# Drexubery/ViewCrafter

Measured on NVIDIA H100. Metric: DDIM denoise-steps/sec @ 576x1024x25f, higher is better.
Workload: dtype f16 (fp32 accumulate; fp32 norms/softmax/update)

## Files before the change

viewcrafter_b200/csrc/common.cuh:

```cuda
#pragma once
#include <cuda.h>
#include <cuda_fp16.h>
#include <cuda_runtime.h>
#include <stdint.h>

#define VC_OK 0
#define VC_ERR_ARG 1
#define VC_ERR_CUDA 2
#define VC_ERR_UNSUPPORTED 3

namespace vc {

void set_error(const char* fmt, ...);
const char* last_error();

#define VC_CHECK_CUDA(expr)                                                                      \
  do {                                                                                           \
    cudaError_t _e = (expr);                                                                     \
    if (_e != cudaSuccess) {                                                                     \
      vc::set_error("%s failed: %s (%s:%d)", #expr, cudaGetErrorString(_e), __FILE__, __LINE__); \
      return VC_ERR_CUDA;                                                                        \
    }                                                                                            \
  } while (0)

#define VC_REQUIRE(cond, ...)       \
  do {                              \
    if (!(cond)) {                  \
      vc::set_error(__VA_ARGS__);   \
      return VC_ERR_ARG;            \
    }                               \
  } while (0)

int encode_tmap_f16(CUtensorMap* out, const void* base, int rank, const uint64_t* dims,
                    const uint64_t* strides_bytes, const uint32_t* box, int swizzle_bytes = 128);

int sm_count();

struct DeviceOnce {
  unsigned long long done[4] = {0, 0, 0, 0};
};
bool device_once_needed(DeviceOnce& o);
void device_once_mark(DeviceOnce& o);

#ifdef __CUDACC__

__device__ __forceinline__ uint32_t smem_u32(const void* p) { return (uint32_t)__cvta_generic_to_shared(p); }

__device__ __forceinline__ bool elect_one() {
  uint32_t pred = 0;
  asm volatile(
      "{\n\t.reg .pred P1;\n\t.reg .b32 R1;\n\t"
      "elect.sync R1|P1, 0xffffffff;\n\t"
      "selp.b32 %0, 1, 0, P1;\n\t}\n"
      : "=r"(pred));
  return pred != 0;
}

__device__ __forceinline__ void mbar_init(uint64_t* bar, uint32_t count) {
  asm volatile("mbarrier.init.shared::cta.b64 [%0], %1;" ::"r"(smem_u32(bar)), "r"(count) : "memory");
}
__device__ __forceinline__ void fence_barrier_init() {
  asm volatile("fence.mbarrier_init.release.cluster;" ::: "memory");
}
__device__ __forceinline__ void fence_proxy_async() {
  asm volatile("fence.proxy.async.shared::cta;" ::: "memory");
}
__device__ __forceinline__ void mbar_expect_tx(uint64_t* bar, uint32_t bytes) {
  asm volatile("mbarrier.arrive.expect_tx.shared::cta.b64 _, [%0], %1;" ::"r"(smem_u32(bar)), "r"(bytes) : "memory");
}
__device__ __forceinline__ void mbar_arrive(uint64_t* bar) {
  asm volatile("mbarrier.arrive.shared::cta.b64 _, [%0];" ::"r"(smem_u32(bar)) : "memory");
}
__device__ __forceinline__ bool mbar_try_wait(uint64_t* bar, uint32_t parity) {
  uint32_t ok;
  asm volatile(
      "{\n\t.reg .pred P1;\n\t"
      "mbarrier.try_wait.parity.shared::cta.b64 P1, [%1], %2;\n\t"
      "selp.b32 %0, 1, 0, P1;\n\t}\n"
      : "=r"(ok)
      : "r"(smem_u32(bar)), "r"(parity)
      : "memory");
  return ok != 0;
}
__device__ __forceinline__ void mbar_wait(uint64_t* bar, uint32_t parity) {
  while (!mbar_try_wait(bar, parity)) {
  }
}
__device__ __forceinline__ void tma_prefetch_desc(const CUtensorMap* m) {
  asm volatile("prefetch.tensormap [%0];" ::"l"(reinterpret_cast<uint64_t>(m)) : "memory");
}
__device__ __forceinline__ void tma_load_2d(void* dst, const CUtensorMap* m, uint64_t* bar, int c0, int c1) {
  asm volatile(
      "cp.async.bulk.tensor.2d.shared::cta.global.mbarrier::complete_tx::bytes [%0], [%1, {%3, %4}], [%2];" ::"r"(smem_u32(dst)),
      "l"(reinterpret_cast<uint64_t>(m)), "r"(smem_u32(bar)), "r"(c0), "r"(c1)
      : "memory");
}
__device__ __forceinline__ void tma_load_4d(void* dst, const CUtensorMap* m, uint64_t* bar, int c0, int c1, int c2, int c3) {
  asm volatile(
      "cp.async.bulk.tensor.4d.shared::cta.global.mbarrier::complete_tx::bytes [%0], [%1, {%3, %4, %5, %6}], [%2];" ::"r"(smem_u32(dst)),
      "l"(reinterpret_cast<uint64_t>(m)), "r"(smem_u32(bar)), "r"(c0), "r"(c1), "r"(c2), "r"(c3)
      : "memory");
}
__device__ __forceinline__ void tma_store_4d(const CUtensorMap* m, const void* src, int c0, int c1, int c2, int c3) {
  asm volatile("cp.async.bulk.tensor.4d.global.shared::cta.bulk_group [%0, {%2, %3, %4, %5}], [%1];" ::"l"(reinterpret_cast<uint64_t>(m)),
               "r"(smem_u32(src)), "r"(c0), "r"(c1), "r"(c2), "r"(c3)
               : "memory");
}
__device__ __forceinline__ void tma_store_3d(const CUtensorMap* m, const void* src, int c0, int c1, int c2) {
  asm volatile("cp.async.bulk.tensor.3d.global.shared::cta.bulk_group [%0, {%2, %3, %4}], [%1];" ::"l"(reinterpret_cast<uint64_t>(m)),
               "r"(smem_u32(src)), "r"(c0), "r"(c1), "r"(c2)
               : "memory");
}
__device__ __forceinline__ void tma_store_commit() { asm volatile("cp.async.bulk.commit_group;" ::: "memory"); }
__device__ __forceinline__ void tma_store_wait_read() { asm volatile("cp.async.bulk.wait_group.read 0;" ::: "memory"); }
__device__ __forceinline__ void tma_store_wait_all() { asm volatile("cp.async.bulk.wait_group 0;" ::: "memory"); }
__device__ __forceinline__ void fence_proxy_async_smem() { asm volatile("fence.proxy.async.shared::cta;" ::: "memory"); }

__device__ __forceinline__ void wgmma_fence() { asm volatile("wgmma.fence.sync.aligned;" ::: "memory"); }
__device__ __forceinline__ void wgmma_commit() { asm volatile("wgmma.commit_group.sync.aligned;" ::: "memory"); }
template <int N>
__device__ __forceinline__ void wgmma_wait() { asm volatile("wgmma.wait_group.sync.aligned %0;" ::"n"(N) : "memory"); }
template <int R>
__device__ __forceinline__ void wgmma_fence_regs(float (&d)[R]) {
#pragma unroll
  for (int i = 0; i < R; ++i) asm volatile("" : "+f"(d[i])::"memory");
}
__device__ __forceinline__ void named_bar_sync(int id, int count) { asm volatile("bar.sync %0, %1;" ::"r"(id), "r"(count) : "memory"); }

__device__ __forceinline__ uint64_t wgmma_desc_sw128(uint32_t smem_addr, uint32_t lbo_bytes = 16, uint32_t sbo_bytes = 1024) {
  uint64_t d = 0;
  d |= (uint64_t)((smem_addr & 0x3FFFF) >> 4);
  d |= (uint64_t)((lbo_bytes >> 4) & 0x3FFF) << 16;
  d |= (uint64_t)((sbo_bytes >> 4) & 0x3FFF) << 32;
  d |= (uint64_t)1 << 62;
  return d;
}

__device__ __forceinline__ uint32_t pack_half2(float a, float b) {
  __half2 h = __floats2half2_rn(a, b);
  return *reinterpret_cast<uint32_t*>(&h);
}

__device__ __forceinline__ float silu_f(float x) { return __fdividef(x, 1.0f + __expf(-x)); }
__device__ __forceinline__ float erf_fast(float x) {
  const float ax = fabsf(x);
  const float t = __frcp_rn(fmaf(0.3275911f, ax, 1.0f));
  float poly = fmaf(1.061405429f, t, -1.453152027f);
  poly = fmaf(poly, t, 1.421413741f);
  poly = fmaf(poly, t, -0.284496736f);
  poly = fmaf(poly, t, 0.254829592f);
  const float y = 1.0f - poly * t * __expf(-ax * ax);
  return copysignf(y, x);
}
__device__ __forceinline__ float gelu_erf_fast(float x) { return 0.5f * x * (1.0f + erf_fast(x * 0.70710678118654752440f)); }
__device__ __forceinline__ float gelu_erf_f(float x) { return 0.5f * x * (1.0f + erff(x * 0.70710678118654752440f)); }

#endif

}
```

viewcrafter_b200/csrc/gemm_common.cuh:

```cuda
#pragma once
#include "common.cuh"

namespace vc {

static constexpr int BM = 128;
static constexpr int BK = 64;
static constexpr int MAX_TAPS = 9;
static constexpr int MMA_WGS = 2;
static constexpr int GEMM_THREADS = 128 * (1 + MMA_WGS);
static constexpr int EPI_WARPS = 4 * MMA_WGS;
static constexpr int EPI_STAGE_BYTES = 32 * 32 * 2;
static constexpr int EPI_XPOSE_PITCH = 72;
static constexpr int EPI_XPOSE_BYTES = 64 * EPI_XPOSE_PITCH * 4;
static constexpr int EPI_SMEM_BYTES = EPI_WARPS * EPI_STAGE_BYTES + MMA_WGS * EPI_XPOSE_BYTES;

struct FastDiv {
  uint32_t mul, shr, d;
};
static inline FastDiv make_fastdiv(int d) {
  FastDiv f;
  f.d = (uint32_t)d;
  if (d == 1) { f.mul = 0; f.shr = 0; return f; }
  uint32_t lg = 0;
  while ((1u << lg) < (uint32_t)d) ++lg;
  const uint32_t p = 31 + lg;
  f.mul = (uint32_t)(((1ull << p) + (uint32_t)d - 1) / (uint32_t)d);
  f.shr = p - 32;
  return f;
}
#ifdef __CUDACC__
__device__ __forceinline__ int fast_div(const FastDiv& f, int n) { return f.d == 1 ? n : (int)(__umulhi((uint32_t)n, f.mul) >> f.shr); }
#endif

static constexpr int GEMM_PEER_MAX = 4;
struct GemmPeer {
  int mode;
  int P, me;
  int wrap;
  int HW, HWl, T, Tl_me;
  int rps;
  FastDiv div_hwl, div_rps, div_tl;
  int f0[GEMM_PEER_MAX + 1];
  CUtensorMap map[GEMM_PEER_MAX];
};

struct GemmParams {
  CUtensorMap tmap_a;
  CUtensorMap tmap_a2;
  CUtensorMap tmap_b;
  CUtensorMap tmap_out;
  int tiles_x, tiles_y, Z;
  FastDiv div_tiles_x, div_tiles_y, div_n_tiles;
  int bx, by;
  int bx_shift;
  int X, Y;
  int N, K, K1;
  int num_taps;
  int tap_dx[MAX_TAPS];
  int tap_dy[MAX_TAPS];
  int n_tiles;
  int total_tiles;
  __half* out;
  float* out_f32;
  int ldo;
  const float* bias;
  int bias_z_div;
  const __half* res;
  int ldr;
  int geglu;
  const float* ln_stats;
  const float* ln_colsum;
  float2* ln_part;
  long long ln_rows;
  float2* gn_part;
  int gn_hp;
  int gn_nchunks;
  int out_tma;
  int vec_ok;
  GemmPeer peer;
};

struct TileCoord {
  int x0, y0, z;
};

#ifdef __CUDACC__
__device__ __forceinline__ TileCoord tile_coord_m(const GemmParams& p, int m) {
  TileCoord t;
  const int q1 = fast_div(p.div_tiles_x, m);
  const int tx = m - q1 * p.tiles_x;
  t.z = fast_div(p.div_tiles_y, q1);
  const int ty = q1 - t.z * p.tiles_y;
  t.x0 = tx << p.bx_shift;
  t.y0 = ty * p.by;
  return t;
}
#endif

#ifdef __CUDACC__
__device__ __forceinline__ float gelu_epilogue(float x) {
  const float z = x * 0.70710678118654752440f;
  const float az = fabsf(z);
  float t;
  asm("rcp.approx.ftz.f32 %0, %1;" : "=f"(t) : "f"(fmaf(0.3275911f, az, 1.0f)));
  float poly = fmaf(1.061405429f, t, -1.453152027f);
  poly = fmaf(poly, t, 1.421413741f);
  poly = fmaf(poly, t, -0.284496736f);
  poly = fmaf(poly, t, 0.254829592f);
  float e;
  asm("ex2.approx.ftz.f32 %0, %1;" : "=f"(e) : "f"(az * az * -1.4426950408889634f));
  const float erf_abs = fmaf(-poly * t, e, 1.0f);
  const float hx = 0.5f * x;
  return fmaf(hx, copysignf(erf_abs, z), hx);
}

struct EpiTile {
  long long orow;
  const float* bias;
  int n_tile;
  int m_tile;
  int quad;
  int wx, wy, wz;
  bool row_ok;
};

__device__ __forceinline__ EpiTile epi_tile(const GemmParams& p, int tile, int quad, int lane) {
  EpiTile t;
  const int mq = fast_div(p.div_n_tiles, tile);
  t.n_tile = tile - mq * p.n_tiles;
  t.m_tile = mq;
  t.quad = quad;
  const TileCoord tc = tile_coord_m(p, t.m_tile);
  const int R = quad * 32 + lane;
  const int R0 = quad * 32;
  t.wx = tc.x0 + (R0 & (p.bx - 1)); t.wy = tc.y0 + (R0 >> p.bx_shift); t.wz = tc.z;
  const int x = tc.x0 + (R & (p.bx - 1)), y = tc.y0 + (R >> p.bx_shift);
  t.row_ok = x < p.X && y < p.Y && tc.z < p.Z;
  t.orow = ((long long)tc.z * p.Y + y) * p.X + x;
  t.bias = p.bias ? p.bias + (long long)(p.bias_z_div > 0 ? min(tc.z, p.Z - 1) / p.bias_z_div : 0) * p.N : nullptr;
  return t;
}

__device__ __forceinline__ void peer_scatter32(const GemmParams& p, const EpiTile& t, int col0, const uint8_t* stage) {
  const GemmPeer& g = p.peer;
  int lin = t.wy * p.X + t.wx;
  int slab = t.wz;
  if (g.wrap) { slab = fast_div(g.div_rps, lin); lin -= slab * g.rps; }
  int rem = 32, i0 = 0;
  while (rem > 0) {
    if (lin >= g.rps) {
      if (!g.wrap) break;
      lin -= g.rps; ++slab;
    }
    int q, s, c2;
    if (g.mode == 1) {
      q = fast_div(g.div_hwl, lin); s = lin - q * g.HWl;
      const int b = fast_div(g.div_tl, slab);
      c2 = b * g.T + g.f0[g.me] + (slab - b * g.Tl_me);
    } else {
      const int tt = fast_div(g.div_hwl, lin); s = lin - tt * g.HWl;
      q = 0;
      while (q + 1 < g.P && tt >= g.f0[q + 1]) ++q;
      c2 = slab * (g.f0[q + 1] - g.f0[q]) + tt - g.f0[q];
    }
    const int len = min(rem, g.HWl - s);
    if (q < g.P) tma_store_3d(&g.map[q], stage, col0, s - i0, c2);
    i0 += len; lin += len; rem -= len;
  }
}

__device__ __forceinline__ void epi_store32(const GemmParams& p, const EpiTile& t, int col0, int n_out, float (&f)[32], bool res_scalar,
                                            uint8_t* stage, int lane) {
  if (p.out_tma) {
    if (lane == 0) tma_store_wait_read();
    __syncwarp();
    const uint32_t sbase = smem_u32(stage) + lane * 64;
    const int sw = (lane >> 1) & 3;
#pragma unroll
    for (int h = 0; h < 4; ++h) {
      const uint32_t u0 = pack_half2(f[h * 8 + 0], f[h * 8 + 1]), u1 = pack_half2(f[h * 8 + 2], f[h * 8 + 3]);
      const uint32_t u2 = pack_half2(f[h * 8 + 4], f[h * 8 + 5]), u3 = pack_half2(f[h * 8 + 6], f[h * 8 + 7]);
      asm volatile("st.shared.v4.b32 [%0], {%1, %2, %3, %4};" ::"r"(sbase + ((h ^ sw) << 4)), "r"(u0), "r"(u1), "r"(u2), "r"(u3) : "memory");
    }
    fence_proxy_async_smem();
    __syncwarp();
    if (lane == 0) {
      if (p.peer.mode) peer_scatter32(p, t, col0, stage);
      else tma_store_4d(&p.tmap_out, stage, col0, t.wx, t.wy, t.wz);
      tma_store_commit();
    }
    return;
  }
  if (!t.row_ok || col0 >= n_out) return;
  if (col0 + 32 <= n_out && p.vec_ok) {
    if (p.out_f32) {
      float4* op = reinterpret_cast<float4*>(p.out_f32 + t.orow * p.ldo + col0);
#pragma unroll
      for (int h = 0; h < 8; ++h) op[h] = make_float4(f[h * 4], f[h * 4 + 1], f[h * 4 + 2], f[h * 4 + 3]);
    } else {
      uint4* op = reinterpret_cast<uint4*>(p.out + t.orow * p.ldo + col0);
#pragma unroll
      for (int h = 0; h < 4; ++h)
        op[h] = make_uint4(pack_half2(f[h * 8 + 0], f[h * 8 + 1]), pack_half2(f[h * 8 + 2], f[h * 8 + 3]), pack_half2(f[h * 8 + 4], f[h * 8 + 5]),
                           pack_half2(f[h * 8 + 6], f[h * 8 + 7]));
    }
  } else {
#pragma unroll
    for (int e = 0; e < 32; ++e) {
      if (col0 + e < n_out) {
        float v = f[e];
        if (res_scalar) v += __half2float(p.res[t.orow * p.ldr + col0 + e]);
        if (p.out_f32) p.out_f32[t.orow * p.ldo + col0 + e] = v;
        else p.out[t.orow * p.ldo + col0 + e] = __float2half_rn(v);
      }
    }
  }
}

template <int B1, int HP>
__device__ __forceinline__ void gn_piece_sums(const float (&f)[32], bool row_ok, float (&v)[8]) {
  float s[4], q[4];
#pragma unroll
  for (int i = 0; i < 4; ++i) s[i] = q[i] = 0.f;
#pragma unroll
  for (int e = 0; e < 16; ++e) {
    const int piece = e < B1 ? 0 : e < B1 + HP ? 1 : e < B1 + 2 * HP ? 2 : 3;
    const float2 r = __half22float2(__floats2half2_rn(f[2 * e], f[2 * e + 1]));
    s[piece] += r.x + r.y;
    q[piece] = fmaf(r.x, r.x, fmaf(r.y, r.y, q[piece]));
  }
#pragma unroll
  for (int i = 0; i < 4; ++i) {
    v[i] = row_ok ? s[i] : 0.f;
    v[4 + i] = row_ok ? q[i] : 0.f;
  }
}
__device__ __forceinline__ void gn_part_accumulate(const GemmParams& p, const EpiTile& t, int nb, const float (&f)[32], int lane) {
  float v[8];
  const int sub = 2 * p.gn_hp;
  const int o = nb % sub;
  if (p.gn_hp == 5) {
    switch (o) {
      case 0: gn_piece_sums<5, 5>(f, t.row_ok, v); break;
      case 2: gn_piece_sums<4, 5>(f, t.row_ok, v); break;
      case 4: gn_piece_sums<3, 5>(f, t.row_ok, v); break;
      case 6: gn_piece_sums<2, 5>(f, t.row_ok, v); break;
      default: gn_piece_sums<1, 5>(f, t.row_ok, v); break;
    }
  } else {
    gn_piece_sums<4, 4>(f, t.row_ok, v);
  }
  {
    const bool hi = lane & 16;
#pragma unroll
    for (int i = 0; i < 4; ++i) {
      const float send = hi ? v[i] : v[i + 4], keep = hi ? v[i + 4] : v[i];
      v[i] = keep + __shfl_xor_sync(0xffffffffu, send, 16);
    }
  }
  {
    const bool hi = lane & 8;
#pragma unroll
    for (int i = 0; i < 2; ++i) {
      const float send = hi ? v[i] : v[i + 2], keep = hi ? v[i + 2] : v[i];
      v[i] = keep + __shfl_xor_sync(0xffffffffu, send, 8);
    }
  }
  {
    const bool hi = lane & 4;
    const float send = hi ? v[0] : v[1], keep = hi ? v[1] : v[0];
    v[0] = keep + __shfl_xor_sync(0xffffffffu, send, 4);
  }
  v[0] += __shfl_xor_sync(0xffffffffu, v[0], 2);
  v[0] += __shfl_xor_sync(0xffffffffu, v[0], 1);
  if ((lane & 3) == 0) {
    const int idx = ((lane >> 4) & 1) * 4 + ((lane >> 3) & 1) * 2 + ((lane >> 2) & 1);
    const long long rb = (long long)t.m_tile * 4 + t.quad;
    float* dst = reinterpret_cast<float*>(p.gn_part + (rb * p.gn_nchunks + (nb >> 5)) * 4);
    dst[(idx & 3) * 2 + (idx >> 2)] = v[0];
  }
}

__device__ __forceinline__ void epi_chunk(const GemmParams& p, const EpiTile& t, int nb, int col0, int n_out, bool plain, float (&f)[32],
                                          uint8_t* stage, int lane) {
  bool res_vec = false;
  if (!plain) {
    if (p.ln_stats) {
      const float2 ln = t.row_ok ? __ldg(reinterpret_cast<const float2*>(p.ln_stats) + t.orow) : make_float2(0.f, 1.f);
#pragma unroll
      for (int e = 0; e < 32; e += 4) {
        const float4 cs = __ldg(reinterpret_cast<const float4*>(p.ln_colsum + nb + e));
        f[e] = (f[e] - ln.x * cs.x) * ln.y; f[e + 1] = (f[e + 1] - ln.x * cs.y) * ln.y;
        f[e + 2] = (f[e + 2] - ln.x * cs.z) * ln.y; f[e + 3] = (f[e + 3] - ln.x * cs.w) * ln.y;
      }
    }
    if (t.bias) {
      if (nb + 32 <= p.N) {
#pragma unroll
        for (int e = 0; e < 32; e += 4) {
          const float4 b4 = __ldg(reinterpret_cast<const float4*>(t.bias + nb + e));
          f[e] += b4.x; f[e + 1] += b4.y; f[e + 2] += b4.z; f[e + 3] += b4.w;
        }
      } else {
#pragma unroll
        for (int e = 0; e < 32; ++e)
          if (nb + e < p.N) f[e] += __ldg(t.bias + nb + e);
      }
    }
    res_vec = p.res != nullptr && p.vec_ok && t.row_ok && nb + 32 <= p.N;
    if (res_vec) {
      const uint4* rp = reinterpret_cast<const uint4*>(p.res + t.orow * p.ldr + nb);
#pragma unroll
      for (int h = 0; h < 4; ++h) {
        const uint4 u = rp[h];
        const __half2* r2 = reinterpret_cast<const __half2*>(&u);
#pragma unroll
        for (int e = 0; e < 4; ++e) {
          const float2 r = __half22float2(r2[e]);
          f[h * 8 + 2 * e] += r.x; f[h * 8 + 2 * e + 1] += r.y;
        }
      }
    }
    if (p.ln_part) {
      float s = 0.f, q = 0.f;
#pragma unroll
      for (int e = 0; e < 32; e += 2) {
        const float2 r = __half22float2(__floats2half2_rn(f[e], f[e + 1]));
        s += r.x + r.y;
        q = fmaf(r.x, r.x, fmaf(r.y, r.y, q));
      }
      if (t.row_ok) p.ln_part[(long long)(nb >> 5) * p.ln_rows + t.orow] = make_float2(s, q);
    }
    if (p.gn_part) gn_part_accumulate(p, t, nb, f, lane);
  }
  epi_store32(p, t, col0, n_out, f, !plain && p.res != nullptr && !res_vec, stage, lane);
}
#endif

}
```

viewcrafter_b200/csrc/gemm_tap.cu:

```cuda
#include "gemm_common.cuh"
#include "kernels.h"
#include "wgmma.cuh"

namespace vc {

template <int BN>
struct GemmCfg {
  static constexpr int A_BYTES = BM * BK * 2;
  static constexpr int B_BYTES = BN * BK * 2;
  static constexpr int STAGE_BYTES = A_BYTES + B_BYTES;
  static constexpr int BUDGET = 227 * 1024 - 1024  - 256  - EPI_SMEM_BYTES;
  static constexpr int STAGES = BUDGET / STAGE_BYTES > 8 ? 8 : BUDGET / STAGE_BYTES;
  static constexpr int SMEM_BYTES = STAGES * STAGE_BYTES + EPI_SMEM_BYTES + 1024 + 256;
  static_assert(STAGES >= 4, "pipeline too shallow");
  static_assert(B_BYTES % 1024 == 0, "stages must stay 1024-byte aligned (128B swizzle atoms)");
};

template <int BN, int NCOLS>
__device__ __forceinline__ void epi_drain(const GemmParams& p, const EpiTile& t, float (&acc)[BN / 2], float* xpose, int cw, int wl, int lane,
                                          uint8_t* stage, bool plain, int nb0, int col0, int n_out) {
  constexpr int SLABS = (NCOLS + 63) / 64;
  const int fr = 16 * wl + (lane >> 2), fc = 2 * (lane & 3);
#pragma unroll
  for (int sl = 0; sl < SLABS; ++sl) {
    named_bar_sync(1 + cw, 128);
#pragma unroll
    for (int jj = 0; jj < 8; ++jj) {
      const int j = sl * 8 + jj;
      if (j < NCOLS / 8) {
        float* d0 = xpose + fr * EPI_XPOSE_PITCH + jj * 8 + fc;
        *reinterpret_cast<float2*>(d0) = make_float2(acc[j * 4], acc[j * 4 + 1]);
        *reinterpret_cast<float2*>(d0 + 8 * EPI_XPOSE_PITCH) = make_float2(acc[j * 4 + 2], acc[j * 4 + 3]);
      }
    }
    named_bar_sync(1 + cw, 128);
    const int c = sl * 2 + (wl >> 1);
    if (c * 32 < NCOLS && (plain ? col0 + c * 32 < n_out : nb0 + c * 32 < p.N)) {
      float f[32];
      const float4* src = reinterpret_cast<const float4*>(xpose + ((wl & 1) * 32 + lane) * EPI_XPOSE_PITCH + (wl >> 1) * 32);
#pragma unroll
      for (int e = 0; e < 8; ++e) {
        const float4 v = src[e];
        f[4 * e] = v.x; f[4 * e + 1] = v.y; f[4 * e + 2] = v.z; f[4 * e + 3] = v.w;
      }
      epi_chunk(p, t, nb0 + c * 32, col0 + c * 32, n_out, plain, f, stage, lane);
    }
  }
}

template <int BN>
__global__ void __launch_bounds__(GEMM_THREADS, 1) gemm_tap_kernel(const __grid_constant__ GemmParams p) {
  using Cfg = GemmCfg<BN>;
  constexpr int STAGES = Cfg::STAGES;
  extern __shared__ uint8_t smem_raw[];
  uint8_t* smem = reinterpret_cast<uint8_t*>((reinterpret_cast<uintptr_t>(smem_raw) + 1023) & ~uintptr_t(1023));
  uint8_t* epi_smem = smem + STAGES * Cfg::STAGE_BYTES;
  uint64_t* full_bar = reinterpret_cast<uint64_t*>(epi_smem + EPI_SMEM_BYTES);
  uint64_t* empty_bar = full_bar + STAGES;

  const int warp = threadIdx.x >> 5;
  const int lane = threadIdx.x & 31;
  const int kblocks = (p.K + BK - 1) / BK;
  const int iters = p.num_taps * kblocks;

  if (threadIdx.x == 0) {
    tma_prefetch_desc(&p.tmap_a);
    tma_prefetch_desc(&p.tmap_b);
    if (p.out_tma) tma_prefetch_desc(&p.tmap_out);
    for (int s = 0; s < STAGES; ++s) {
      mbar_init(&full_bar[s], 1);
      mbar_init(&empty_bar[s], EPI_WARPS);
    }
    fence_barrier_init();
  }
  __syncthreads();

  if (warp == 0) {
    int s = 0;
    uint32_t ph = 0;
    for (int tile = blockIdx.x; tile < p.total_tiles; tile += gridDim.x) {
      const int m_tile = fast_div(p.div_n_tiles, tile);
      const TileCoord tc = tile_coord_m(p, m_tile);
      const int n0 = (tile - m_tile * p.n_tiles) * BN;
      for (int tap = 0; tap < p.num_taps; ++tap) {
        const int cx = tc.x0 + p.tap_dx[tap], cy = tc.y0 + p.tap_dy[tap];
        const int brow = tap * p.N + n0;
        for (int kb = 0; kb < kblocks; ++kb) {
          mbar_wait(&empty_bar[s], ph ^ 1);
          if (elect_one()) {
            uint8_t* sa = smem + s * Cfg::STAGE_BYTES;
            uint8_t* sb = sa + Cfg::A_BYTES;
            mbar_expect_tx(&full_bar[s], Cfg::STAGE_BYTES);
            const int k = kb * BK;
            if (k < p.K1)
              tma_load_4d(sa, &p.tmap_a, &full_bar[s], k, cx, cy, tc.z);
            else
              tma_load_4d(sa, &p.tmap_a2, &full_bar[s], k - p.K1, cx, cy, tc.z);
            tma_load_2d(sb, &p.tmap_b, &full_bar[s], k, brow);
          }
          __syncwarp();
          if (++s == STAGES) { s = 0; ph ^= 1; }
        }
      }
    }
  } else if (warp >= 4) {
    const int cw = (warp >> 2) - 1;
    const int wl = warp & 3;
    uint8_t* stage = epi_smem + (warp - 4) * EPI_STAGE_BYTES;
    float* xpose = reinterpret_cast<float*>(epi_smem + EPI_WARPS * EPI_STAGE_BYTES + cw * EPI_XPOSE_BYTES);
    const uint32_t ring = smem_u32(smem);
    float acc[BN / 2];
#pragma unroll
    for (int i = 0; i < BN / 2; ++i) acc[i] = 0.f;
    int s = 0;
    uint32_t ph = 0;
    for (int tile = blockIdx.x; tile < p.total_tiles; tile += gridDim.x) {
      int prev = -1;
      for (int i = 0; i < iters; ++i) {
        mbar_wait(&full_bar[s], ph);
        const uint32_t a_addr = ring + s * Cfg::STAGE_BYTES + cw * (64 * BK * 2);
        const uint32_t b_addr = ring + s * Cfg::STAGE_BYTES + Cfg::A_BYTES;
        wgmma_fence();
#pragma unroll
        for (int k = 0; k < BK / 16; ++k)
          Wgmma<BN>::ss(acc, wgmma_desc_sw128(a_addr + 32 * k), wgmma_desc_sw128(b_addr + 32 * k), (i > 0 || k > 0) ? 1 : 0);
        wgmma_commit();
        wgmma_wait<1>();
        if (prev >= 0) {
          __syncwarp();
          if (lane == 0) mbar_arrive(&empty_bar[prev]);
        }
        prev = s;
        if (++s == STAGES) { s = 0; ph ^= 1; }
      }
      wgmma_wait<0>();
      wgmma_fence_regs(acc);
      if (prev >= 0) {
        __syncwarp();
        if (lane == 0) mbar_arrive(&empty_bar[prev]);
      }
      const EpiTile t = epi_tile(p, tile, cw * 2 + (wl & 1), lane);
      const int n0 = t.n_tile * BN;
      if (!p.geglu) {
        epi_drain<BN, BN>(p, t, acc, xpose, cw, wl, lane, stage, false, n0, n0, p.N);
      } else {
        constexpr int HALF = BN / 2;
        const TileCoord tc = tile_coord_m(p, t.m_tile);
        float2 ln[2] = {make_float2(0.f, 1.f), make_float2(0.f, 1.f)};
        if (p.ln_stats) {
#pragma unroll
          for (int h = 0; h < 2; ++h) {
            const int R = cw * 64 + 16 * wl + (lane >> 2) + 8 * h;
            const int x = tc.x0 + (R & (p.bx - 1)), y = tc.y0 + (R >> p.bx_shift);
            if (x < p.X && y < p.Y && tc.z < p.Z)
              ln[h] = __ldg(reinterpret_cast<const float2*>(p.ln_stats) + ((long long)tc.z * p.Y + y) * p.X + x);
          }
        }
#pragma unroll
        for (int j = 0; j < HALF / 8; ++j) {
#pragma unroll
          for (int e = 0; e < 4; ++e) {
            const int n = n0 + 8 * j + 2 * (lane & 3) + (e & 1);
            float a = acc[j * 4 + e], g = acc[(j + HALF / 8) * 4 + e];
            if (p.ln_stats) {
              const float2 l = ln[e >> 1];
              a = (a - l.x * __ldg(p.ln_colsum + n)) * l.y;
              g = (g - l.x * __ldg(p.ln_colsum + n + HALF)) * l.y;
            }
            if (t.bias) { a += __ldg(t.bias + n); g += __ldg(t.bias + n + HALF); }
            acc[j * 4 + e] = a * gelu_epilogue(g);
          }
        }
        epi_drain<BN, HALF>(p, t, acc, xpose, cw, wl, lane, stage, true, n0, t.n_tile * HALF, p.N / 2);
      }
    }
    if (p.out_tma && lane == 0) tma_store_wait_all();
  }
}

template <int BN>
static int launch_gemm(const GemmParams& p, cudaStream_t stream) {
  using Cfg = GemmCfg<BN>;
  static DeviceOnce configured;
  if (device_once_needed(configured)) {
    VC_CHECK_CUDA(cudaFuncSetAttribute(gemm_tap_kernel<BN>, cudaFuncAttributeMaxDynamicSharedMemorySize, Cfg::SMEM_BYTES));
    device_once_mark(configured);
  }
  const int grid = p.total_tiles < sm_count() ? p.total_tiles : sm_count();
  gemm_tap_kernel<BN><<<grid, GEMM_THREADS, Cfg::SMEM_BYTES, stream>>>(p);
  VC_CHECK_CUDA(cudaGetLastError());
  return VC_OK;
}

static int pick_bn(int N, int geglu) {
  if (geglu) return 128;
  if (N <= 32) return 32;
  if (N <= 64) return 64;
  if (N % 160 == 0) return 160;
  if (N % 128 == 0) return 128;
  if (N % 96 == 0 && N <= 192) return 96;
  if (N % 64 == 0 && N < 256) return 64;
  return 128;
}

int pick_bn_public(int N, int geglu) { return pick_bn(N, geglu); }

int gemm_tap(const GemmDesc& d, cudaStream_t stream) {
  VC_REQUIRE(d.a && d.w && (d.out || d.out_f32), "gemm_tap: null pointer");
  VC_REQUIRE(d.num_taps >= 1 && d.num_taps <= MAX_TAPS, "gemm_tap: num_taps=%d out of range", d.num_taps);
  VC_REQUIRE(d.bx * d.by == BM && d.bx >= 1, "gemm_tap: box %dx%d must cover 128 rows", d.bx, d.by);
  VC_REQUIRE(d.by == 1 || d.bx == d.X, "gemm_tap: multi-row boxes need bx == X (X=%d bx=%d)", d.X, d.bx);
  VC_REQUIRE(d.K % 8 == 0 && d.lda % 8 == 0, "gemm_tap: K and lda must be multiples of 8 (TMA 16-byte strides)");
  VC_REQUIRE(d.K1 == d.K || (d.a2 && d.K1 % BK == 0 && d.K1 < d.K), "gemm_tap: bad K split K1=%d K=%d", d.K1, d.K);
  VC_REQUIRE(!d.geglu || (d.N % 128 == 0 && !d.res && !d.out_f32), "gemm_tap: GEGLU needs N %% 128 == 0");
  if ((reinterpret_cast<uintptr_t>(d.a) & 15) || (reinterpret_cast<uintptr_t>(d.w) & 15)) {
    set_error("gemm_tap: operands must be 16-byte aligned");
    return VC_ERR_ARG;
  }
  const void* optr = d.out_f32 ? (const void*)d.out_f32 : (const void*)d.out;
  const int esz = d.out_f32 ? 4 : 2;

  GemmParams p;
  memset(&p, 0, sizeof(p));
  const int BN = pick_bn(d.N, d.geglu);
  p.bx = d.bx; p.by = d.by; p.X = d.X; p.Y = d.Y; p.Z = d.Z;
  p.tiles_x = (d.X + d.bx - 1) / d.bx;
  p.tiles_y = (d.Y + d.by - 1) / d.by;
  p.n_tiles = (d.N + BN - 1) / BN;
  p.div_tiles_x = make_fastdiv(p.tiles_x);
  p.div_tiles_y = make_fastdiv(p.tiles_y);
  p.div_n_tiles = make_fastdiv(p.n_tiles);
  p.bx_shift = 0;
  while ((1 << p.bx_shift) < d.bx) ++p.bx_shift;
  VC_REQUIRE((1 << p.bx_shift) == d.bx, "gemm_tap: bx=%d must be a power of two", d.bx);
  const long long m_tiles = (long long)p.tiles_x * p.tiles_y * p.Z;

  {
    uint64_t dims[4] = {(uint64_t)d.K1, (uint64_t)d.X, (uint64_t)d.Y, (uint64_t)d.Z};
    uint64_t str[3] = {(uint64_t)d.lda * 2, (uint64_t)d.lda * 2 * d.X, (uint64_t)d.lda * 2 * d.X * d.Y};
    uint32_t box[4] = {(uint32_t)BK, (uint32_t)d.bx, (uint32_t)d.by, 1};
    int rc = encode_tmap_f16(&p.tmap_a, d.a, 4, dims, str, box);
    if (rc) return rc;
    if (d.K1 != d.K) {
      uint64_t dims2[4] = {(uint64_t)(d.K - d.K1), (uint64_t)d.X, (uint64_t)d.Y, (uint64_t)d.Z};
      uint64_t str2[3] = {(uint64_t)d.lda2 * 2, (uint64_t)d.lda2 * 2 * d.X, (uint64_t)d.lda2 * 2 * d.X * d.Y};
      rc = encode_tmap_f16(&p.tmap_a2, d.a2, 4, dims2, str2, box);
      if (rc) return rc;
    } else {
      p.tmap_a2 = p.tmap_a;
    }
  }
  {
    uint64_t dims[2] = {(uint64_t)d.K, (uint64_t)d.num_taps * d.N};
    uint64_t str[1] = {(uint64_t)(d.ldw > 0 ? d.ldw : d.K) * 2};
    uint32_t box[2] = {(uint32_t)BK, (uint32_t)BN};
    int rc = encode_tmap_f16(&p.tmap_b, d.w, 2, dims, str, box);
    if (rc) return rc;
  }
  p.N = d.N; p.K = d.K; p.K1 = d.K1;
  p.num_taps = d.num_taps;
  for (int t = 0; t < d.num_taps; ++t) { p.tap_dx[t] = d.tap_dx[t]; p.tap_dy[t] = d.tap_dy[t]; }
  p.out = d.out; p.out_f32 = d.out_f32; p.ldo = d.ldo;
  p.bias = d.bias; p.bias_z_div = d.bias_z_div;
  p.res = d.res; p.ldr = d.ldr;
  p.geglu = d.geglu;
  VC_REQUIRE((d.ln_stats == nullptr) == (d.ln_colsum == nullptr), "gemm_tap: ln_stats and ln_colsum go together");
  VC_REQUIRE(!d.ln_stats || (d.num_taps == 1 && d.N % 32 == 0 && d.Y == 1 && d.Z == 1 && !d.a2),
             "gemm_tap: folded LayerNorm needs a plain [M,K] x [N,K] GEMM with N %% 32 == 0");
  VC_REQUIRE(!d.ln_stats || ((reinterpret_cast<uintptr_t>(d.ln_stats) & 7) == 0 && (reinterpret_cast<uintptr_t>(d.ln_colsum) & 15) == 0),
             "gemm_tap: ln_stats / ln_colsum misaligned");
  p.ln_stats = d.ln_stats; p.ln_colsum = d.ln_colsum;
  VC_REQUIRE(!d.ln_part || (d.num_taps == 1 && d.N % 32 == 0 && d.Y == 1 && d.Z == 1 && !d.geglu && d.out && !d.out_f32 &&
                            (reinterpret_cast<uintptr_t>(d.ln_part) & 7) == 0),
             "gemm_tap: LayerNorm partial sums need a plain fp16 [M,N] output with N %% 32 == 0");
  p.ln_part = reinterpret_cast<float2*>(d.ln_part); p.ln_rows = d.X;
  VC_REQUIRE(!d.gn_part || ((d.gn_sub == 10 || d.gn_sub == 8) && d.N % 32 == 0 && d.N % d.gn_sub == 0 && !d.geglu && d.out && !d.out_f32 &&
                            (reinterpret_cast<uintptr_t>(d.gn_part) & 7) == 0),
             "gemm_tap: GroupNorm partial sums need an fp16 output with N %% 32 == 0 and N %% gn_sub == 0 (gn_sub 10 or 8)");
  p.gn_part = reinterpret_cast<float2*>(d.gn_part); p.gn_hp = d.gn_sub / 2; p.gn_nchunks = d.N / 32;
  const bool o_al = ((reinterpret_cast<uintptr_t>(optr) & 31) == 0) && ((long long)d.ldo * esz) % 32 == 0;
  const bool r_al = !d.res || (((reinterpret_cast<uintptr_t>(d.res) & 31) == 0) && ((long long)d.ldr * 2) % 32 == 0);
  p.vec_ok = (o_al && r_al) ? 1 : 0;
  {
    const int n_out = d.geglu ? d.N / 2 : d.N;
    p.out_tma = (d.out && !d.out_f32 && n_out % 32 == 0 && (reinterpret_cast<uintptr_t>(d.out) & 15) == 0 && d.ldo % 8 == 0) ? 1 : 0;
    if (p.out_tma) {
      const uint32_t bw = d.bx < 32 ? d.bx : 32;
      uint64_t dims[4] = {(uint64_t)n_out, (uint64_t)d.X, (uint64_t)d.Y, (uint64_t)d.Z};
      const long long py = d.ldo_y > 0 ? d.ldo_y : (long long)d.ldo * d.X;
      const long long pz = d.ldo_z > 0 ? d.ldo_z : py * d.Y;
      uint64_t str[3] = {(uint64_t)d.ldo * 2, (uint64_t)py * 2, (uint64_t)pz * 2};
      uint32_t box[4] = {32, bw, 32 / bw, 1};
      int rc = encode_tmap_f16(&p.tmap_out, d.out, 4, dims, str, box, 64);
      if (rc) return rc;
    }
    VC_REQUIRE((d.ldo_y == 0 && d.ldo_z == 0) || (p.out_tma && !d.res && !d.ln_part),
               "gemm_tap: strided (ldo_y / ldo_z) outputs need the TMA-store epilogue (fp16, N %% 32 == 0) and no residual");
  }
  if (d.peer && d.peer->mode) {
    const GemmPeerDesc& q = *d.peer;
    VC_REQUIRE(q.mode == 1 || q.mode == 2, "gemm_tap: peer mode %d", q.mode);
    VC_REQUIRE(q.world >= 2 && q.world <= GEMM_PEER_MAX && q.rank >= 0 && q.rank < q.world, "gemm_tap: peer scatter supports 2..%d ranks", GEMM_PEER_MAX);
    VC_REQUIRE(p.out_tma && !d.geglu && !d.ln_part && d.ldo_y == 0 && d.ldo_z == 0, "gemm_tap: peer scatter needs the fp16 TMA-store epilogue");
    VC_REQUIRE(q.HW % q.world == 0 && q.f0[0] == 0 && q.f0[q.world] == q.T && q.B >= 1, "gemm_tap: peer scatter: bad frame / site split");
    GemmPeer& g = p.peer;
    g.mode = q.mode; g.P = q.world; g.me = q.rank;
    g.HW = q.HW; g.HWl = q.HW / q.world; g.T = q.T;
    g.Tl_me = q.f0[q.rank + 1] - q.f0[q.rank];
    for (int r = 0; r <= q.world; ++r) g.f0[r] = q.f0[r];
    const long long rows = (long long)d.X * d.Y * d.Z;
    g.rps = q.mode == 1 ? q.HW : q.T * g.HWl;
    VC_REQUIRE(rows == (q.mode == 1 ? (long long)q.B * g.Tl_me * q.HW : (long long)q.B * q.T * g.HWl), "gemm_tap: peer scatter: %lld rows do not match the layout", rows);
    const bool row_major_patches = d.Y == 1 || d.bx == d.X || (d.by == 1 && d.X % 32 == 0);
    VC_REQUIRE(row_major_patches && (d.bx >= 32 || 32 % d.bx == 0), "gemm_tap: peer scatter: tile box %dx%d of a %dx%d image is not row-contiguous", d.bx, d.by, d.X, d.Y);
    if (d.Y == 1 && d.Z == 1) { g.wrap = 1; }
    else { g.wrap = 0; VC_REQUIRE((long long)d.X * d.Y == g.rps, "gemm_tap: peer scatter: slab of %d rows expected, tile geometry has %lld", g.rps, (long long)d.X * d.Y); }
    g.div_hwl = make_fastdiv(g.HWl); g.div_rps = make_fastdiv(g.rps); g.div_tl = make_fastdiv(g.Tl_me > 0 ? g.Tl_me : 1);
    for (int r = 0; r < q.world; ++r) {
      VC_REQUIRE(q.dst[r] && (reinterpret_cast<uintptr_t>(q.dst[r]) & 15) == 0, "gemm_tap: peer scatter: destination %d missing / misaligned", r);
      const int tl_r = q.f0[r + 1] - q.f0[r];
      const __half* base = reinterpret_cast<const __half*>(q.dst[r]) + (q.mode == 2 ? (long long)q.rank * g.HWl * d.N : 0);
      uint64_t dims[3] = {(uint64_t)d.N, (uint64_t)g.HWl, (uint64_t)(q.mode == 1 ? (long long)q.B * q.T : (long long)q.B * tl_r)};
      if (dims[2] == 0) dims[2] = 1;
      uint64_t str[2] = {(uint64_t)d.N * 2, (uint64_t)(q.mode == 1 ? g.HWl : q.HW) * d.N * 2};
      uint32_t box[3] = {32, 32, 1};
      int rc = encode_tmap_f16(&g.map[r], base, 3, dims, str, box, 64);
      if (rc) return rc;
    }
  }
  const long long total = m_tiles * p.n_tiles;
  VC_REQUIRE(total > 0 && total < (1ll << 31), "gemm_tap: tile count %lld out of range", total);
  p.total_tiles = (int)total;
  switch (BN) {
    case 32: return launch_gemm<32>(p, stream);
    case 64: return launch_gemm<64>(p, stream);
    case 96: return launch_gemm<96>(p, stream);
    case 128: return launch_gemm<128>(p, stream);
    case 160: return launch_gemm<160>(p, stream);
  }
  set_error("gemm_tap: no kernel for BN=%d", BN);
  return VC_ERR_UNSUPPORTED;
}

}
```

Measured before the change: 1.791.

## Ping-pong consumer warpgroups over whole tiles with register reallocation

Each MMA warpgroup now computes a full 128-row tile into two accumulator halves and alternates tiles with the other warpgroup. Named barriers order their mainloops so one group's epilogue overlaps the other's MMA. Producer warps give up registers via setmaxnreg so the consumers can hold the doubled accumulators. This costs more register pressure and more complex barrier and phase bookkeeping, and it needs a launch-bounds register count consistent with the split.

```diff
diff --git a/viewcrafter_b200/csrc/common.cuh b/viewcrafter_b200/csrc/common.cuh
--- a/viewcrafter_b200/csrc/common.cuh
+++ b/viewcrafter_b200/csrc/common.cuh
@@ -126,6 +126,11 @@
   for (int i = 0; i < R; ++i) asm volatile("" : "+f"(d[i])::"memory");
 }
 __device__ __forceinline__ void named_bar_sync(int id, int count) { asm volatile("bar.sync %0, %1;" ::"r"(id), "r"(count) : "memory"); }
+__device__ __forceinline__ void named_bar_arrive(int id, int count) { asm volatile("bar.arrive %0, %1;" ::"r"(id), "r"(count) : "memory"); }
+template <int R>
+__device__ __forceinline__ void setmaxnreg_dec() { asm volatile("setmaxnreg.dec.sync.aligned.u32 %0;" ::"n"(R)); }
+template <int R>
+__device__ __forceinline__ void setmaxnreg_inc() { asm volatile("setmaxnreg.inc.sync.aligned.u32 %0;" ::"n"(R)); }
 
 __device__ __forceinline__ uint64_t wgmma_desc_sw128(uint32_t smem_addr, uint32_t lbo_bytes = 16, uint32_t sbo_bytes = 1024) {
   uint64_t d = 0;
diff --git a/viewcrafter_b200/csrc/gemm_common.cuh b/viewcrafter_b200/csrc/gemm_common.cuh
--- a/viewcrafter_b200/csrc/gemm_common.cuh
+++ b/viewcrafter_b200/csrc/gemm_common.cuh
@@ -8,6 +8,10 @@
 static constexpr int MAX_TAPS = 9;
 static constexpr int MMA_WGS = 2;
 static constexpr int GEMM_THREADS = 128 * (1 + MMA_WGS);
+static constexpr int GEMM_LAUNCH_REGS = 168;
+static constexpr int GEMM_PRODUCER_REGS = 24;
+static constexpr int GEMM_MMA_REGS = 240;
+static_assert(128 * GEMM_PRODUCER_REGS + 128 * MMA_WGS * GEMM_MMA_REGS <= GEMM_LAUNCH_REGS * GEMM_THREADS, "register split exceeds the CTA's allocation");
 static constexpr int EPI_WARPS = 4 * MMA_WGS;
 static constexpr int EPI_STAGE_BYTES = 32 * 32 * 2;
 static constexpr int EPI_XPOSE_PITCH = 72;
diff --git a/viewcrafter_b200/csrc/gemm_tap.cu b/viewcrafter_b200/csrc/gemm_tap.cu
--- a/viewcrafter_b200/csrc/gemm_tap.cu
+++ b/viewcrafter_b200/csrc/gemm_tap.cu
@@ -69,13 +69,15 @@
     if (p.out_tma) tma_prefetch_desc(&p.tmap_out);
     for (int s = 0; s < STAGES; ++s) {
       mbar_init(&full_bar[s], 1);
-      mbar_init(&empty_bar[s], EPI_WARPS);
+      mbar_init(&empty_bar[s], 4);
     }
     fence_barrier_init();
   }
   __syncthreads();
 
-  if (warp == 0) {
+  if (warp < 4) {
+    setmaxnreg_dec<GEMM_PRODUCER_REGS>();
+    if (warp != 0) return;
     int s = 0;
     uint32_t ph = 0;
     for (int tile = blockIdx.x; tile < p.total_tiles; tile += gridDim.x) {
@@ -103,27 +105,40 @@
         }
       }
     }
-  } else if (warp >= 4) {
+  } else {
+    setmaxnreg_inc<GEMM_MMA_REGS>();
     const int cw = (warp >> 2) - 1;
     const int wl = warp & 3;
     uint8_t* stage = epi_smem + (warp - 4) * EPI_STAGE_BYTES;
     float* xpose = reinterpret_cast<float*>(epi_smem + EPI_WARPS * EPI_STAGE_BYTES + cw * EPI_XPOSE_BYTES);
     const uint32_t ring = smem_u32(smem);
-    float acc[BN / 2];
-#pragma unroll
-    for (int i = 0; i < BN / 2; ++i) acc[i] = 0.f;
+    float acc[2][BN / 2];
+#pragma unroll
+    for (int h = 0; h < 2; ++h)
+#pragma unroll
+      for (int i = 0; i < BN / 2; ++i) acc[h][i] = 0.f;
     int s = 0;
     uint32_t ph = 0;
-    for (int tile = blockIdx.x; tile < p.total_tiles; tile += gridDim.x) {
+    auto skip_tile = [&]() {
+      s += iters;
+      ph ^= (uint32_t)(s / STAGES) & 1u;
+      s %= STAGES;
+    };
+    if (cw == 1) skip_tile();
+    for (int tile = blockIdx.x + cw * gridDim.x; tile < p.total_tiles; tile += 2 * gridDim.x) {
+      if (tile >= (int)gridDim.x) named_bar_sync(3 + cw, 256);
       int prev = -1;
       for (int i = 0; i < iters; ++i) {
         mbar_wait(&full_bar[s], ph);
-        const uint32_t a_addr = ring + s * Cfg::STAGE_BYTES + cw * (64 * BK * 2);
+        const uint32_t a_addr = ring + s * Cfg::STAGE_BYTES;
         const uint32_t b_addr = ring + s * Cfg::STAGE_BYTES + Cfg::A_BYTES;
         wgmma_fence();
 #pragma unroll
-        for (int k = 0; k < BK / 16; ++k)
-          Wgmma<BN>::ss(acc, wgmma_desc_sw128(a_addr + 32 * k), wgmma_desc_sw128(b_addr + 32 * k), (i > 0 || k > 0) ? 1 : 0);
+        for (int k = 0; k < BK / 16; ++k) {
+          const uint64_t db = wgmma_desc_sw128(b_addr + 32 * k);
+          Wgmma<BN>::ss(acc[0], wgmma_desc_sw128(a_addr + 32 * k), db, (i > 0 || k > 0) ? 1 : 0);
+          Wgmma<BN>::ss(acc[1], wgmma_desc_sw128(a_addr + 64 * BK * 2 + 32 * k), db, (i > 0 || k > 0) ? 1 : 0);
+        }
         wgmma_commit();
         wgmma_wait<1>();
         if (prev >= 0) {
@@ -133,45 +148,51 @@
         prev = s;
         if (++s == STAGES) { s = 0; ph ^= 1; }
       }
+      if (tile + (int)gridDim.x < p.total_tiles) named_bar_arrive(4 - cw, 256);
+      skip_tile();
       wgmma_wait<0>();
-      wgmma_fence_regs(acc);
+      wgmma_fence_regs(acc[0]);
+      wgmma_fence_regs(acc[1]);
       if (prev >= 0) {
         __syncwarp();
         if (lane == 0) mbar_arrive(&empty_bar[prev]);
       }
-      const EpiTile t = epi_tile(p, tile, cw * 2 + (wl & 1), lane);
-      const int n0 = t.n_tile * BN;
-      if (!p.geglu) {
-        epi_drain<BN, BN>(p, t, acc, xpose, cw, wl, lane, stage, false, n0, n0, p.N);
-      } else {
-        constexpr int HALF = BN / 2;
-        const TileCoord tc = tile_coord_m(p, t.m_tile);
-        float2 ln[2] = {make_float2(0.f, 1.f), make_float2(0.f, 1.f)};
-        if (p.ln_stats) {
-#pragma unroll
-          for (int h = 0; h < 2; ++h) {
-            const int R = cw * 64 + 16 * wl + (lane >> 2) + 8 * h;
-            const int x = tc.x0 + (R & (p.bx - 1)), y = tc.y0 + (R >> p.bx_shift);
-            if (x < p.X && y < p.Y && tc.z < p.Z)
-              ln[h] = __ldg(reinterpret_cast<const float2*>(p.ln_stats) + ((long long)tc.z * p.Y + y) * p.X + x);
+#pragma unroll
+      for (int h = 0; h < 2; ++h) {
+        const EpiTile t = epi_tile(p, tile, h * 2 + (wl & 1), lane);
+        const int n0 = t.n_tile * BN;
+        if (BN != 128 || !p.geglu) {
+          epi_drain<BN, BN>(p, t, acc[h], xpose, cw, wl, lane, stage, false, n0, n0, p.N);
+        } else {
+          constexpr int HALF = BN / 2;
+          const TileCoord tc = tile_coord_m(p, t.m_tile);
+          float2 ln[2] = {make_float2(0.f, 1.f), make_float2(0.f, 1.f)};
+          if (p.ln_stats) {
+#pragma unroll
+            for (int r = 0; r < 2; ++r) {
+              const int R = h * 64 + 16 * wl + (lane >> 2) + 8 * r;
+              const int x = tc.x0 + (R & (p.bx - 1)), y = tc.y0 + (R >> p.bx_shift);
+              if (x < p.X && y < p.Y && tc.z < p.Z)
+                ln[r] = __ldg(reinterpret_cast<const float2*>(p.ln_stats) + ((long long)tc.z * p.Y + y) * p.X + x);
+            }
           }
+#pragma unroll
+          for (int j = 0; j < HALF / 8; ++j) {
+#pragma unroll
+            for (int e = 0; e < 4; ++e) {
+              const int n = n0 + 8 * j + 2 * (lane & 3) + (e & 1);
+              float a = acc[h][j * 4 + e], g = acc[h][(j + HALF / 8) * 4 + e];
+              if (p.ln_stats) {
+                const float2 l = ln[e >> 1];
+                a = (a - l.x * __ldg(p.ln_colsum + n)) * l.y;
+                g = (g - l.x * __ldg(p.ln_colsum + n + HALF)) * l.y;
+              }
+              if (t.bias) { a += __ldg(t.bias + n); g += __ldg(t.bias + n + HALF); }
+              acc[h][j * 4 + e] = a * gelu_epilogue(g);
+            }
+          }
+          epi_drain<BN, HALF>(p, t, acc[h], xpose, cw, wl, lane, stage, true, n0, t.n_tile * HALF, p.N / 2);
         }
-#pragma unroll
-        for (int j = 0; j < HALF / 8; ++j) {
-#pragma unroll
-          for (int e = 0; e < 4; ++e) {
-            const int n = n0 + 8 * j + 2 * (lane & 3) + (e & 1);
-            float a = acc[j * 4 + e], g = acc[(j + HALF / 8) * 4 + e];
-            if (p.ln_stats) {
-              const float2 l = ln[e >> 1];
-              a = (a - l.x * __ldg(p.ln_colsum + n)) * l.y;
-              g = (g - l.x * __ldg(p.ln_colsum + n + HALF)) * l.y;
-            }
-            if (t.bias) { a += __ldg(t.bias + n); g += __ldg(t.bias + n + HALF); }
-            acc[j * 4 + e] = a * gelu_epilogue(g);
-          }
-        }
-        epi_drain<BN, HALF>(p, t, acc, xpose, cw, wl, lane, stage, true, n0, t.n_tile * HALF, p.N / 2);
       }
     }
     if (p.out_tma && lane == 0) tma_store_wait_all();
```

Result: faster. 1.857, median of 6 (+3.7%).
